# CycloneBoy/pdf_table

Measured on AMD Instinct MI355X. Metric: pages/s, higher is better.
Workload: dtype bf16

## Files before the change

### include/pdftable_hip.h

```cpp
#ifndef PDFTABLE_HIP_H
#define PDFTABLE_HIP_H

#include <stddef.h>
#include <stdint.h>

#ifdef __cplusplus
extern "C" {
#endif

#define PT_OK 0
#define PT_ERR_INVALID 1
#define PT_ERR_HIP 2
#define PT_ERR_STATE 3
#define PT_ERR_FORMAT 4

typedef struct pt_engine pt_engine;
typedef void* pt_stream;

int pt_engine_create(int device_id, pt_engine** out);
void pt_engine_destroy(pt_engine* e);
const char* pt_last_error(void);
int pt_abi_version(void);
int pt_engine_check(pt_engine* e);
int pt_engine_set_lstm_cluster(pt_engine* e, int on);
// ... 170 lines not shown
                 pt_stream stream);
int pt_op_conv1x1_ex(pt_engine* e, const uint16_t* d_in, int B, int H, int W, int Cin, const uint16_t* d_w_tiled, const float* d_bias,
                     int N, uint16_t* d_out, float* d_out_f32, int out_cstride, int n_valid, const float* d_res_f32, int relu,
                     const int32_t* d_ylimit, pt_stream stream);

int pt_op_dcn(pt_engine* e, const uint16_t* d_in, const float* d_om, int B, int H, int W, int C, const uint16_t* d_w_tiled,
              const float* d_bias, int N, uint16_t* d_out, int relu, int split, pt_stream stream);

int pt_op_stem7x7(pt_engine* e, const uint16_t* d_in, int B, int H, int W, const uint16_t* d_w, const float* d_bias,
                  uint16_t* d_out, int split, pt_stream stream);
int pt_op_maxpool3x3s2(pt_engine* e, const uint16_t* d_in, int B, int H, int W, int C, uint16_t* d_out, int split,
                       pt_stream stream);
int pt_op_db_head_final(pt_engine* e, const uint16_t* d_in, int B, int H, int W, const void* d_w, const float* d_bias,
                        float* d_prob, float* d_logits, int split, pt_stream stream);

int pt_op_dwconv(pt_engine* e, const uint16_t* d_in, int B, int H, int W, int C, const float* d_w_taps, const float* d_bias, int k,
                 int stride, int act, uint16_t* d_out, int split, pt_stream stream);
int pt_op_add(pt_engine* e, const uint16_t* d_a, const uint16_t* d_b, uint16_t* d_out, long long npix, int C, int split, pt_stream stream);
int pt_op_maxpool(pt_engine* e, const uint16_t* d_in, int B, int H, int W, int C, int k, int stride, int pad, uint16_t* d_out,
                  int split, pt_stream stream);
int pt_op_avgpool(pt_engine* e, const uint16_t* d_in, int B, int H, int W, int C, int k, uint16_t* d_out, int split, pt_stream stream);
int pt_op_chan_mean(pt_engine* e, const uint16_t* d_in, int B, int HW, int C, float* d_scratch, uint16_t* d_mean, int split, pt_stream stream);
int pt_op_chan_mean_scratch_floats(int B, int C);
int pt_op_scale_channels(pt_engine* e, const uint16_t* d_in, const uint16_t* d_gate, int B, int HW, int C, uint16_t* d_out,
                         int split, pt_stream stream);
int pt_op_act(pt_engine* e, const uint16_t* d_in, long long n_elems, int kind, float alpha, float beta, uint16_t* d_out, int C, int split,
              pt_stream stream);
int pt_op_copy_channels(pt_engine* e, const uint16_t* d_src, long long npix, int src_cstride, int src_coff, uint16_t* d_dst, int dst_cstride, int dst_coff,
                        int n, pt_stream stream);
int pt_op_upsample_nearest(pt_engine* e, const uint16_t* d_in, int B, int H, int W, int C, int factor, uint16_t* d_out, pt_stream stream);
int pt_op_mul(pt_engine* e, const uint16_t* d_a, const uint16_t* d_b, uint16_t* d_out, long long n_elems, int C, int split, pt_stream stream);
int pt_copy_bytes(pt_engine* e, const void* src, void* dst, long long nbytes, pt_stream stream);
int pt_op_layernorm(pt_engine* e, const uint16_t* d_in, long long rows, int c_pad, int c, const float* d_gamma, const float* d_beta, float eps,
                    uint16_t* d_out, int split, pt_stream stream);
int pt_op_softmax(pt_engine* e, const uint16_t* d_in, long long rows, int c_pad, int c, float* d_out_f32, uint16_t* d_out_bf16, int split, pt_stream stream);
int pt_op_attention(pt_engine* e, const uint16_t* d_qkv, int B, int T, int heads, int d, int qkv_cstride, float scale, uint16_t* d_out, int out_cstride,
                    int split, pt_stream stream);

#define PT_CLS_SLOTS 4
#define PT_CLS_MAX_CLASSES 16
typedef struct pt_cls_image {
  int64_t offset;
  int32_t h, w;
} pt_cls_image;

int pt_cls_preprocess(pt_engine* e, const uint8_t* d_base, const pt_cls_image* d_images, int n, int max_h, int max_w,
// ... 50 lines not shown
```

### pdf_table_amd/csrc/api_common.cpp

```cpp
#include <stdarg.h>
#include <stdio.h>

#include "../../include/pdftable_hip.h"

static thread_local char g_err[1024] = "";

void pt_set_error(const char* fmt, ...) {
  va_list ap;
  va_start(ap, fmt);
  vsnprintf(g_err, sizeof(g_err), fmt, ap);
  va_end(ap);
}

extern "C" {

const char* pt_last_error(void) { return g_err; }

int pt_abi_version(void) { return 16; }

}
```

### pdf_table_amd/csrc/c_api.hip

```cpp
#include <stdarg.h>
#include <stdio.h>
#include <stdlib.h>

#include <cmath>

#include "common.h"

namespace PT_FMT_NS {
namespace api {

static int ensure(void** buf, size_t* cap, size_t need);

int pt_engine_check(pt_engine* e) {
  PT_REQUIRE(e, "pt_engine_check: null engine");
  if (e->lstm_err && *e->lstm_err) {
    *e->lstm_err = 0;
    e->lstm_cluster = 0;
    pt_set_error("lstm_cluster_kernel: a workgroup waited > 2^22 polls for its peers -- the launch was not co-resident "
                 "(GPU shared with another process or stream?).  The recognition results since the last check are invalid; "
                 "this engine now uses the streaming LSTM kernel (pt_engine_set_lstm_cluster(e, 0)): run the batch again");
    return PT_ERR_HIP;
  }
  return PT_OK;
}
// ... 910 lines not shown
                 const float* d_bias, int N, int ks, int stride, uint16_t* d_out, int out_cstride, int out_coff,
                 int rep, int shuffle_cout, const uint16_t* d_res, int res_mode, int relu, int split, int out_lo_off,
                 pt_stream stream) {
  PT_REQUIRE(e != nullptr, "pt_op_conv2d: null engine");
  ConvDesc d;
  d.in = d_in; d.B = B; d.H = H; d.W = W; d.Cin = Cin; d.w = d_w_tiled; d.bias = d_bias; d.N = N; d.ks = ks;
  d.stride = stride; d.out = d_out; d.out_cstride = out_cstride; d.out_coff = out_coff; d.rep = rep;
  d.shuffle_cout = shuffle_cout; d.res = d_res; d.res_mode = res_mode; d.relu = relu;
  d.split = split; d.out_lo_off = out_lo_off;
  return pt_launch_conv(e, d, reinterpret_cast<hipStream_t>(stream));
}

int pt_op_conv1x1_ex(pt_engine* e, const uint16_t* d_in, int B, int H, int W, int Cin, const uint16_t* d_w_tiled, const float* d_bias,
                     int N, uint16_t* d_out, float* d_out_f32, int out_cstride, int n_valid, const float* d_res_f32, int relu,
                     const int32_t* d_ylimit, pt_stream stream) {
  PT_REQUIRE(e != nullptr, "pt_op_conv1x1_ex: null engine");
  ConvDesc d;
  d.in = d_in; d.B = B; d.H = H; d.W = W; d.Cin = Cin; d.w = d_w_tiled; d.bias = d_bias; d.N = N; d.ks = 1; d.stride = 1;
  d.out = d_out_f32 ? nullptr : d_out; d.out_f32 = d_out_f32; d.out_cstride = out_cstride; d.n_valid = n_valid; d.res_f32 = d_res_f32;
  d.relu = relu; d.ylimit = d_ylimit;
  return pt_launch_conv(e, d, reinterpret_cast<hipStream_t>(stream));
}

int pt_op_stem7x7(pt_engine* e, const uint16_t* d_in, int B, int H, int W, const uint16_t* d_w, const float* d_bias,
                  uint16_t* d_out, int split, pt_stream stream) {
  PT_REQUIRE(e != nullptr, "pt_op_stem7x7: null engine");
  return pt_launch_stem7x7(e, d_in, B, H, W, d_w, d_bias, d_out, split, reinterpret_cast<hipStream_t>(stream));
}

int pt_op_maxpool3x3s2(pt_engine* e, const uint16_t* d_in, int B, int H, int W, int C, uint16_t* d_out, int split,
                       pt_stream stream) {
  PT_REQUIRE(e && d_in && d_out, "pt_op_maxpool3x3s2: bad arguments");
  return pt_launch_maxpool3x3s2(d_in, B, H, W, C, d_out, split, reinterpret_cast<hipStream_t>(stream));
}

int pt_op_db_head_final(pt_engine* e, const uint16_t* d_in, int B, int H, int W, const void* d_w, const float* d_bias,
                        float* d_prob, float* d_logits, int split, pt_stream stream) {
  PT_REQUIRE(e && d_in && d_w && d_bias && (d_prob || d_logits), "pt_op_db_head_final: bad arguments");
  return pt_launch_db_head_final(d_in, B, H, W, d_w, d_bias, d_prob, d_logits, split, reinterpret_cast<hipStream_t>(stream));
}

int pt_op_dcn(pt_engine* e, const uint16_t* d_in, const float* d_om, int B, int H, int W, int C, const uint16_t* d_w_tiled,
              const float* d_bias, int N, uint16_t* d_out, int relu, int split, pt_stream stream) {
  PT_REQUIRE(e && d_in && d_om && d_w_tiled && d_bias && d_out, "pt_op_dcn: null argument");
  PT_REQUIRE(B > 0 && H > 0 && W > 0, "pt_op_dcn: empty map (B=%d H=%d W=%d)", B, H, W);
  return pt_launch_dcn_fused(e, d_in, d_om, d_w_tiled, d_bias, d_out, B, H, W, C, N, split, relu, reinterpret_cast<hipStream_t>(stream));
// ... 86 lines not shown
```

### pdf_table_amd/csrc/common.h

```cpp
#pragma once
#include <hip/hip_runtime.h>
#include <stdint.h>
#include <string.h>

#include <map>
#include <string>
#include <vector>

#include "../../include/pdftable_hip.h"
#include "act16.h"

typedef uint16_t bf16_t;

void pt_set_error(const char* fmt, ...);

#define PT_HIP_CHECK(expr)                                                                  \
  do {                                                                                      \
    hipError_t _e = (expr);                                                                 \
    if (_e != hipSuccess) {                                                                 \
      pt_set_error("%s failed: %s (%s:%d)", #expr, hipGetErrorString(_e), __FILE__, __LINE__); \
      return PT_ERR_HIP;                                                                    \
    }                                                                                       \
  } while (0)

// ... 278 lines not shown
  int* cols;
  int* glist;
  int* blist3a;
  int* blist2a;
  int* blist2b;
};
int pt_launch_rows_live_list(const int* lim, int n, int* glist, hipStream_t s);
int pt_launch_crnn_limits(const pt_rec_line* lines, int n, const PtCrnnLimits& L, hipStream_t s);
int pt_launch_crnn_fill(bf16_t* out, const bf16_t* ref, const int* lim, int tile_w, int div, int n, int rows, int W, int cs,
                        hipStream_t s, const int* end_lim = nullptr, int end_tile = 1);
int pt_launch_crnn_conv0_pool(const bf16_t* in, int n, int H, int W, const float* w64x9, const float* bias, int split,
                              bf16_t* out, hipStream_t s, const int* xlim = nullptr);
int pt_launch_maxpool_kxk(const bf16_t* in, int n, int H, int W, int C, int kh, int kw, int h2c, int split, bf16_t* out,
                          hipStream_t s);
int pt_launch_lstm(pt_engine* e, const bf16_t* gx, const bf16_t* whh, bf16_t* hout, int B, int T, int split, hipStream_t s);
int pt_launch_gemm_argmax(const bf16_t* A, long long M, int K, const bf16_t* W, const float* bias, int N, int* ids, float* maxv,
                          hipStream_t s);
int pt_launch_gemm_argmax_x3(const bf16_t* A, long long M, int K, const bf16_t* W3, const float* bias, int N, int n_real, int* ids, float* maxv,
                             void* scratch, hipStream_t s);
int pt_launch_gemm_rows_x3(const bf16_t* A, long long M, int K, const bf16_t* W3, const float* bias, int N, bf16_t* out, int relu, hipStream_t s,
                           const int* tlim = nullptr);
int pt_launch_gemm_rows(const bf16_t* A, long long M, int K, const bf16_t* W, const float* bias, int N, bf16_t* out, int relu,
                        hipStream_t s, const int* tlim = nullptr);
int pt_launch_argmax_reduce(const float* part, long long rows, int ntiles, int* ids, float* maxv, hipStream_t s);
int pt_crnn_forward_net(pt_engine* e, const bf16_t* gray, int n, int32_t* ids, float* maxlogit, hipStream_t s,
                        const pt_rec_line* d_lines = nullptr);

int pt_cvit_forward_net(pt_engine* e, const float* gray, int layout, int n, int32_t* ids, float* maxlogit, hipStream_t s,
                        const int* h_text_w = nullptr);
int pt_launch_rec_resize_gray_f32(const uint8_t* crops, const pt_rec_line* lines, const long long* pix_off, int n_lines, int tw,
                                  float* out, hipStream_t s);

int pt_mtl_backbone_forward_net(pt_engine* e, const bf16_t* x, int n, int H, int W, float* f3, hipStream_t s);
void pt_mtl_release(pt_engine* e);
int pt_mtl_preprocess(pt_engine* e, const uint8_t* pages, int ph, int pw, const pt_tsr_table* tabs, int n, int size, bf16_t* out, hipStream_t s);
int pt_mtl_decoder_config(pt_engine* e, int32_t* out13);
int pt_mtl_structure(pt_engine* e, const float* f3, int n, int hw, float* d_tag_logits, float* d_boxes, int32_t* h_lens, int32_t* h_cell_counts,
                     int force_redecode, hipStream_t s);
int pt_mtl_cells(pt_engine* e, int total, int32_t* d_cell_ids, float* d_cell_prob, float* d_cell_logits, int32_t* h_steps, int force_redecode,
                 hipStream_t s);

int pt_db_forward_net(pt_engine* e, const bf16_t* x, int n, int H, int W, float* prob, float* logits, hipStream_t s, uint32_t* bitmap = nullptr,
                      float thresh = 0.f, int* bitmap_done = nullptr);
int pt_launch_tsr_preprocess(const uint8_t* pages, int ph, int pw, const pt_tsr_table* tabs, int n, int H, int W, int bgr,
                             const float* lut, bf16_t* out, int split, hipStream_t s);
int pt_picodet_forward_net(pt_engine* e, const bf16_t* x, int n, int H, int W, float* h0, float* h1, float* h2, float* h3,
// ... 71 lines not shown
```

### pdf_table_amd/csrc/crnn_model.hip

```cpp
#include <stdlib.h>

#include "common.h"

namespace PT_FMT_NS {

namespace {

struct ConvW {
  const PtTensor *w = nullptr, *b = nullptr;
};

int getw(const PtModel& m, const std::string& base, bool x3, ConvW& out) {
  out.w = m.find(base + (x3 ? ".w3" : ".w"));
  out.b = m.find(base + ".b");
  if (!out.w || !out.b) {
    pt_set_error("CRNN weight blob lacks '%s'", base.c_str());
    return PT_ERR_FORMAT;
  }
  return PT_OK;
}

inline const bf16_t* W(const PtTensor* t) { return reinterpret_cast<const bf16_t*>(t->d_ptr); }
inline const float* Bv(const PtTensor* t) { return reinterpret_cast<const float*>(t->d_ptr); }

// ... 81 lines not shown
#define RUN(call) do { if ((rc = (call)) != PT_OK) return rc; } while (0)
  auto conv = [&](const bf16_t* in, int B, int hh, int ww, int cin, const ConvW& cw, int N, int ks, bf16_t* out, int relu) {
    ConvDesc c;
    c.in = in; c.B = B; c.H = hh; c.W = ww; c.Cin = cin; c.w = W(cw.w); c.bias = Bv(cw.b); c.N = N; c.ks = ks;
    c.stride = 1; c.out = out; c.out_cstride = N * m; c.relu = relu; c.split = x3; c.out_lo_off = N;
    return c;
  };
  static int fused = -1;
  if (fused < 0) {
    const char* ev = getenv("PT_CLS_FUSED");
    fused = ev ? atoi(ev) : 1;
  }
  auto rows_x3 = [&]() {
    const char* ev = getenv("PT_ROWS_X3");
    return x3 && fused && !pt_f16x2(e) && !(ev && ev[0] == '0');
  };
  auto gemm_pipe = [&]() {
    const char* ev = getenv("PT_GEMM_PIPE");
    return !x3 && !(ev && ev[0] == '0');
  };
  auto rows_gemm = [&](const bf16_t* in, int cin, const ConvW& cw, int N, bf16_t* out, int relu, const char* label) -> int {
    if (!x3 && fused && (cin == 256 || (cin == 512 && !gemm_pipe()))) {
      PtProfScope ps(e, s, PT_PROF_CONV1X1, 2.0 * n * T * (double)cin * N, label);
      return pt_launch_gemm_rows(in, (long long)n * T, cin, W(cw.w), Bv(cw.b), N, out, relu, s);
    }
    if (rows_x3() && (cin == 512 || cin == 256)) {
      char lb[48];
      snprintf(lb, sizeof(lb), "%s x3", label);
      PtProfScope ps(e, s, PT_PROF_CONV1X1, 2.0 * n * T * (double)cin * N, lb);
      return pt_launch_gemm_rows_x3(in, (long long)n * T, cin, W(cw.w), Bv(cw.b), N, out, relu, s);
    }
    return pt_launch_conv(e, conv(in, 1, n, T, cin, cw, N, 1, out, relu), s);
  };
  int pool_fused = 1;
  {
    const char* ev = getenv("PT_POOL_FUSED");
    if (ev) pool_fused = atoi(ev);
  }
  auto conv_stack = [&](const bf16_t* g, int nn, bf16_t* a0, bf16_t* a1, bf16_t* p1, bf16_t* c2a_o, bf16_t* c2b_o, bf16_t* p2,
                        bf16_t* c3a_o, bf16_t* c3b_o, bf16_t* p3, bf16_t* f_o, bf16_t* gx_o, const PtCrnnLimits* lim,
                        const bf16_t* zl) -> int {
    auto limited = [&](ConvDesc c, int k) {
      if (lim) {
        c.xlimit = lim->lim[k]; c.xlimit_cols = lim->cols + k;
        if (k == 3) c.block_list = lim->blist3a;
        if (k == 4) c.block_list = lim->glist;
// ... 32 lines not shown
      ConvDesc c2d = limited(conv(c2a_o, nn, 8, 160, 256, c2b, 256, 3, p2, 1), 2);
      c2d.pool = 2;
      RUN(pt_launch_conv(e, c2d, s));
      RUN(fill(p2, ZeroLine::P2, 2, 32, 1, 4, 160, 256, 3, 64));
    } else {
      RUN(pt_launch_conv(e, conv(c2a_o, nn, 8, 160, 256, c2b, 256, 3, c2b_o, 1), s));
      RUN(pt_launch_maxpool_kxk(c2b_o, nn, 8, 160, 256, 2, 1, 0, x3, p2, s));
    }
    RUN(pt_launch_conv(e, limited(conv(p2, nn, 4, 160, 256, c3a, 512, 3, c3a_o, 1), 3), s));
    RUN(fill(c3a_o, ZeroLine::C3A, 3, 32, 1, 4, 160, 512, 4, 64));
    if (pool_fused) {
      ConvDesc c3d = limited(conv(c3a_o, nn, 4, 160, 512, c3b, 512, 3, p3, 1), 4);
      c3d.pool = 3;
      RUN(pt_launch_conv(e, c3d, s));
    } else {
      RUN(pt_launch_conv(e, conv(c3a_o, nn, 4, 160, 512, c3b, 512, 3, c3b_o, 1), s));
      RUN(pt_launch_maxpool_kxk(c3b_o, nn, 4, 160, 512, 2, 1, 1, x3, p3, s));
    }
    {
      ConvDesc c4d = conv(p3, 1, nn, T, 1024, c4, 512, 1, f_o, 1);
      if (lim) { c4d.xlimit_rows = lim->lim[4]; c4d.xlimit_cols = lim->cols + 5; c4d.block_list = lim->glist; }
      RUN(pt_launch_conv(e, c4d, s));
    }
    if ((!x3 && fused && !gemm_pipe()) || rows_x3()) {
      int lim_slot = -1;
      {
        PtProfScope ps(e, s, PT_PROF_CONV1X1, 2.0 * nn * T * 512.0 * 2048, x3 ? "rows gemm 512->2048 x3" : "rows gemm 512->2048");
        if (x3) RUN(pt_launch_gemm_rows_x3(f_o, (long long)nn * T, 512, W(xp1.w), Bv(xp1.b), 2048, gx_o, 0, s, lim ? lim->glist : nullptr));
        else RUN(pt_launch_gemm_rows(f_o, (long long)nn * T, 512, W(xp1.w), Bv(xp1.b), 2048, gx_o, 0, s, lim ? lim->glist : nullptr));
        if (lim && ps.idx >= 0 && e->prof.h_lims && e->prof.n_lims < PtProfile::MAX_LIMS) {
          auto& pd = e->prof.pending[ps.idx];
          pd.lim_slot = lim_slot = e->prof.n_lims++;
          pd.rows = nn * T;
        }
      }
      if (lim_slot >= 0) (void)hipMemcpyAsync(e->prof.h_lims + lim_slot, lim->cols + 5, sizeof(int), hipMemcpyDeviceToHost, s);
    } else {
      ConvDesc xd = conv(f_o, 1, nn, T, 512, xp1, 2048, 1, gx_o, 0);
      if (lim) { xd.xlimit_rows = lim->lim[4]; xd.xlimit_cols = lim->cols + 5; xd.block_list = lim->glist; }
      RUN(pt_launch_conv(e, xd, s));
    }
    RUN(fill(gx_o, ZeroLine::GX, 4, 32, 1, 1, 160, 2048, -1, 1));
    return PT_OK;
  };
  const bool ragged = d_lines != nullptr && pool_fused && e->rec_ragged;
  PtCrnnLimits lim;
  const bf16_t* zl = nullptr;
  if (ragged) {
    if (!e->rec_zero_valid[x3]) {
      const size_t bytes = ZeroLine::END * m * sizeof(bf16_t);
      if (!e->rec_zero[x3]) PT_HIP_CHECK(hipMalloc(&e->rec_zero[x3], bytes));
      PT_HIP_CHECK(hipMemsetAsync(e->rec_zero[x3], 0, bytes, s));
      bf16_t* z = reinterpret_cast<bf16_t*>(e->rec_zero[x3]);
      RUN(conv_stack(z + ZeroLine::GRAY * m, 1, z + ZeroLine::A0 * m, nullptr, z + ZeroLine::P1 * m, z + ZeroLine::C2A * m, nullptr,
                     z + ZeroLine::P2 * m, z + ZeroLine::C3A * m, nullptr, z + ZeroLine::P3 * m, z + ZeroLine::F * m,
                     z + ZeroLine::GX * m, nullptr, nullptr));
      e->rec_zero_valid[x3] = true;
      if (!e->rec_zero_ready[x3]) PT_HIP_CHECK(hipEventCreateWithFlags(&e->rec_zero_ready[x3], hipEventDisableTiming));
      PT_HIP_CHECK(hipEventRecord(e->rec_zero_ready[x3], s));
    } else if (e->rec_zero_ready[x3]) {
      PT_HIP_CHECK(hipStreamWaitEvent(s, e->rec_zero_ready[x3], 0));
    }
    zl = reinterpret_cast<const bf16_t*>(e->rec_zero[x3]);
    const size_t need = ((size_t)26 * n + 40) * sizeof(int);
    if (need > e->rec_limits_cap) {
// ... 57 lines not shown
```

### pdf_table_amd/csrc/rec_kernels.hip

```cpp
#include <math.h>

#include "common.h"

namespace PT_FMT_NS {

typedef __attribute__((ext_vector_type(8))) __bf16 bf16x8;
typedef __attribute__((ext_vector_type(16))) float f32x16;
typedef __attribute__((ext_vector_type(4))) uint32_t u32x4;
typedef __attribute__((ext_vector_type(2))) uint32_t u32x2;

__device__ __forceinline__ float rbf2f(uint32_t bits16) { return a16_to_f32(bits16); }
__device__ __forceinline__ uint32_t rf2bf(float f) { return f32_to_a16(f); }

__global__ __launch_bounds__(256) void rec_warp_kernel(const uint8_t* __restrict__ pages, int ph, int pw,
                                                        const pt_rec_line* __restrict__ lines, int n_lines,
                                                        const long long* __restrict__ pix_off, uint8_t* __restrict__ crops) {
  a16_kernel_enter();
  const int li = blockIdx.y;
  if (li >= n_lines) return;
  const pt_rec_line L = lines[li];
  const int cw = L.crop_w, chh = L.crop_h;
  const long long npx = (long long)cw * chh;
  uint8_t* dst = crops + pix_off[li] * 3;
  const uint8_t* src = pages + (size_t)L.page * ph * pw * 3;
// ... 1900 lines not shown
int pt_launch_gemm_rows(const bf16_t* A, long long M, int K, const bf16_t* W, const float* bias, int N, bf16_t* out, int relu,
                        hipStream_t s, const int* tlim) {
  if ((K != 512 && K != 256) || N % 64 != 0 || M <= 0) return PT_ERR_INVALID;
  const int nw = gemm_nw(4);
  const int smem = 64 * (K * 2 + 16) + 64 * 4 + nw * 32 * 80;
  static bool attr_done = false;
  if (!attr_done) {
    PT_HIP_CHECK(hipFuncSetAttribute(reinterpret_cast<const void*>(&gemm_argmax_kernel<32, 1>), hipFuncAttributeMaxDynamicSharedMemorySize, 64 * (512 * 2 + 16) + 256 + 4 * 32 * 80));
    PT_HIP_CHECK(hipFuncSetAttribute(reinterpret_cast<const void*>(&gemm_argmax_kernel<32, 1, 8>), hipFuncAttributeMaxDynamicSharedMemorySize, 64 * (512 * 2 + 16) + 256 + 8 * 32 * 80));
    attr_done = true;
  }
  const dim3 grid((unsigned)((M + nw * 32 - 1) / (nw * 32))), blk(nw * 64);
  if (K == 512) {
    if (nw == 8) hipLaunchKernelGGL((gemm_argmax_kernel<32, 1, 8>), grid, blk, smem, s, A, M, W, bias, N, nullptr, nullptr, out, relu, tlim, 512, 16ll * 2048);
    else hipLaunchKernelGGL((gemm_argmax_kernel<32, 1>), grid, blk, smem, s, A, M, W, bias, N, nullptr, nullptr, out, relu, tlim, 512, 16ll * 2048);
  } else {
    if (nw == 8) hipLaunchKernelGGL((gemm_argmax_kernel<16, 1, 8>), grid, blk, smem, s, A, M, W, bias, N, nullptr, nullptr, out, relu, tlim, 256, 8ll * 2048);
    else hipLaunchKernelGGL((gemm_argmax_kernel<16, 1>), grid, blk, smem, s, A, M, W, bias, N, nullptr, nullptr, out, relu, tlim, 256, 8ll * 2048);
  }
  PT_HIP_CHECK(hipGetLastError());
  return PT_OK;
}

template <int KSTEPS>
__global__ __launch_bounds__(256, KSTEPS == 32 ? 1 : 2) void gemm_rows_x3_kernel(const bf16_t* __restrict__ A, long long M, const bf16_t* __restrict__ W3,
                                                                                 const float* __restrict__ bias, int N, bf16_t* __restrict__ out, int relu,
                                                                                 const int* __restrict__ tlim) {
  a16_kernel_enter();
  constexpr int K = KSTEPS * 16, NCH = K / 32, P = K * 2 + 16;
  constexpr int NPF = NCH;
  extern __shared__ __attribute__((aligned(16))) char smem[];
  char* sw = smem;
  float* sb = reinterpret_cast<float*>(smem + 64 * P);
  const int tid = threadIdx.x, lane = tid & 63, wave = tid >> 6;
  const int lx = lane & 31, q = lane >> 5;
  long long row0 = ((long long)blockIdx.x * 4 + wave) * 32;
  bool live = row0 < M;
  if (tlim) {
    const int total = tlim[0], g = blockIdx.x * 4 + wave;
    if ((int)blockIdx.x * 4 >= total) return;
    live = g < total;
    row0 = live ? (long long)tlim[1 + g] * 32 : 0;
  }
  const long long row = row0 + lx;
  const long long rc = row < M ? row : M - 1;
  bf16x8 ahi[KSTEPS], alo[KSTEPS];
// ... 112 lines not shown
```

### pdf_table_amd/engine.py

```python
from __future__ import annotations

import contextlib
import ctypes as C
import functools
import threading
from typing import Optional, Sequence, Tuple

import numpy as np
import torch

from . import lib as L

__all__ = ["HipEngine", "REC_LINE_DTYPE", "CLS_IMAGE_DTYPE", "REC_PP_ITEM_DTYPE"]

TSR_TABLE_DTYPE = np.dtype([("minv", "<f8", (6,)), ("page", "<i4"), ("x0", "<i4"), ("y0", "<i4"),
                            ("crop_w", "<i4"), ("crop_h", "<i4"), ("reserved", "<i4")])
CLS_IMAGE_DTYPE = np.dtype([("offset", "<i8"), ("h", "<i4"), ("w", "<i4")])
REC_LINE_DTYPE = np.dtype([("minv", np.float64, (9,)), ("page", np.int32), ("crop_w", np.int32), ("crop_h", np.int32),
                           ("reserved", np.int32)])


REC_PP_ITEM_DTYPE = np.dtype([("line", "<i4"), ("resized_w", "<i4"), ("img_w", "<i4"), ("reserved", "<i4"),
                              ("out_off", "<i8")])

# ... 606 lines not shown
        if out is None:
            if shuffle_cout:
                out = torch.empty((B, 2 * Ho, 2 * Wo, shuffle_cout * m), dtype=self.act_dtype, device=self._tdev)
            else:
                out = torch.empty((B, Ho * rep, Wo * rep, N * m), dtype=self.act_dtype, device=self._tdev)
        L.check(self.lib.pt_op_conv2d(self._h, _ptr(x), B, H, W, Cin, _ptr(w_tiled), _ptr(bias), N, ks, stride,
                                      _ptr(out), out.shape[-1], out_coff, rep, shuffle_cout, _ptr(res), res_mode,
                                      int(relu), int(split), out.shape[-1] // 2, self._stream()), "pt_op_conv2d")
        return out

    def op_conv1x1_ex(self, x: torch.Tensor, w_tiled: torch.Tensor, bias: torch.Tensor, relu: int = 0, out_f32: bool = False,
                      n_valid: int = 0, res_f32: Optional[torch.Tensor] = None, ylimit: Optional[torch.Tensor] = None) -> torch.Tensor:
        self._chk(x, self.act_dtype, "x")
        self._chk(bias, torch.float32, "bias")
        B, H, W, Cin = x.shape
        N = bias.numel()
        cs = n_valid or N
        out = torch.zeros((B, H, W, cs), dtype=torch.float32 if out_f32 else self.act_dtype, device=self._tdev)
        L.check(self.lib.pt_op_conv1x1_ex(self._h, _ptr(x), B, H, W, Cin, _ptr(w_tiled), _ptr(bias), N, None if out_f32 else _ptr(out),
                                          _ptr(out) if out_f32 else None, cs, n_valid, _ptr(res_f32), int(relu), _ptr(ylimit),
                                          self._stream()), "pt_op_conv1x1_ex")
        return out

    def op_dcn(self, x: torch.Tensor, om: torch.Tensor, w_tiled: torch.Tensor, bias: torch.Tensor, relu: bool = True, split: int = 0) -> torch.Tensor:
        self._chk(x, self.act_dtype, "x")
        self._chk(om, torch.float32, "om")
        self._chk(bias, torch.float32, "bias")
        B, H, W, Cc = x.shape
        m = 2 if split else 1
        Cc //= m
        if tuple(om.shape) != (B, H, W, 32):
            raise ValueError(f"op_dcn: om must be [B,H,W,32], got {tuple(om.shape)}")
        N = bias.numel()
        out = torch.empty((B, H, W, N * m), dtype=self.act_dtype, device=self._tdev)
        L.check(self.lib.pt_op_dcn(self._h, _ptr(x), _ptr(om), B, H, W, Cc, _ptr(w_tiled), _ptr(bias), N, _ptr(out), int(relu), int(split),
                                   self._stream()), "pt_op_dcn")
        return out

    def op_dwconv(self, x: torch.Tensor, w_taps: torch.Tensor, bias: torch.Tensor, k: int, stride: int = 1, act: int = 0, split: bool = False) -> torch.Tensor:
        self._chk(x, self.act_dtype, "x")
        self._chk(w_taps, torch.float32, "w_taps")
        self._chk(bias, torch.float32, "bias")
        B, H, W, Cc = x.shape
        pad = k // 2
        out = torch.empty((B, (H + 2 * pad - k) // stride + 1, (W + 2 * pad - k) // stride + 1, Cc), dtype=self.act_dtype, device=self._tdev)
        L.check(self.lib.pt_op_dwconv(self._h, _ptr(x), B, H, W, Cc // 2 if split else Cc, _ptr(w_taps), _ptr(bias), k, stride, act, _ptr(out), int(split),
# ... 258 lines not shown
```

### pdf_table_amd/lib.py

```python
from __future__ import annotations

import ctypes as C
import os

_HERE = os.path.dirname(os.path.abspath(__file__))
LIB_PATH = os.environ.get("PT_LIB_PATH") or os.path.join(_HERE, "libpdftable_hip.so")

PT_MODEL_DB_RESNET18 = 1
PT_MODEL_CRNN = 2
PT_MODEL_LORE_DLA34 = 3
PT_MODEL_LORE_PROCESSOR = 4
PT_MODEL_PICODET = 5
PT_MODEL_LORE_RESNET18 = 6
PT_MODEL_DB_NAS = 7
PT_MODEL_PPLCNET = 8
PT_MODEL_CONVNEXT_VIT = 16
PT_MODEL_MTL_BACKBONE = 17
PT_MODEL_MTL_DECODER = 18
PT_MODEL_CENTERNET_DLA34 = 19
PT_CVIT_W, PT_CVIT_CHUNK_W, PT_CVIT_CHUNK_STEP, PT_CVIT_T, PT_CVIT_NCLS = 804, 300, 252, 201, 7644
PT_CLS_SLOTS = 4
PT_CLS_MAX_CLASSES = 16
PT_LAYOUT_HEAD_CS, PT_LAYOUT_CAND_FLOATS = 40, 48
PT_DET_PRE_DB_PP = 0
PT_DET_PRE_DB_TORCH = 1
PT_DET_PRE_NONE = 2
PT_PRECISION_BF16 = 0
PT_PRECISION_BF16X3 = 1
PT_PRECISION_F16X2 = 2
PT_PRECISION_F16 = 3
PT_DET_POST_DB_PP = 0
PT_DET_POST_DB_TORCH = 1
PT_TSR_MAX_CELLS = 3000
PT_CENTERNET_MAX_CELLS = 1000
PT_ROTATE_90_CLOCKWISE, PT_ROTATE_180, PT_ROTATE_90_COUNTERCLOCKWISE = 0, 1, 2
PT_REC_H, PT_REC_W, PT_REC_T, PT_REC_NCLS = 32, 640, 160, 7644
PT_PROF_CLASSES = ("conv3x3", "conv1x1", "stem", "other")
EXPECTED_ABI = 16

_lib = None


class PtError(RuntimeError):
    pass


def _proto(lib):
    vp, i, f, sz = C.c_void_p, C.c_int, C.c_float, C.c_size_t
    ip = C.POINTER(C.c_int)
    P = {
        "pt_engine_create": (i, [i, C.POINTER(vp)]),
        "pt_engine_destroy": (None, [vp]),
        "pt_last_error": (C.c_char_p, []),
        "pt_abi_version": (i, []),
        "pt_engine_check": (i, [vp]),
        "pt_engine_set_precision": (i, [vp, i]),
        "pt_engine_set_lstm_cluster": (i, [vp, i]),
        "pt_engine_set_mtl_kv_fp8": (i, [vp, i]),
        "pt_engine_set_dcn_mfma": (i, [vp, i]),
        "pt_weights_load": (i, [vp, i, vp, sz]),
        "pt_weights_load_device": (i, [vp, i, vp, sz, vp]),
# ... 30 lines not shown
        "pt_layout_forward": (i, [vp, vp, i, i, i, i, i, i, f, i, vp, vp, vp]),
        "pt_tsr_preprocess": (i, [vp, vp, i, i, i, vp, i, i, i, i, vp, vp]),
        "pt_tsr_forward_net": (i, [vp, vp, i, i, i, vp, vp, vp, vp, vp, vp, vp]),
        "pt_tsr_forward_net_wireless": (i, [vp, vp, i, i, i, vp, vp, vp, vp, vp, vp, vp]),
        "pt_tsr_decode": (i, [vp, vp, vp, vp, vp, vp, vp, i, i, i, i, f, vp, vp, vp, vp]),
        "pt_tsr_forward_decode": (i, [vp, vp, i, i, i, i, f, vp, vp, vp, vp]),
        "pt_tsr_process": (i, [vp, vp, vp, vp, i, i, vp, vp, vp]),
        "pt_centernet_forward_net": (i, [vp, vp, i, i, i, vp, vp, vp, vp, vp]),
        "pt_centernet_decode": (i, [vp, vp, vp, vp, vp, i, i, i, vp, vp, vp, vp]),
        "pt_hard_nms": (i, [vp, vp, vp, i, C.c_double, i, vp, vp]),
        "pt_page_line_mask": (i, [vp, i, i, i, vp, vp]),
        "pt_page_line_angles": (i, [vp, i, i, i, i, i, vp, i, vp]),
        "pt_page_warp_cubic": (i, [vp, i, i, i, vp, vp, i, vp, vp]),
        "pt_page_quarter_turn": (i, [vp, i, i, i, i, vp, vp]),
        "pt_page_pre_tables": (i, [vp, vp]),
        "pt_cls_preprocess": (i, [vp, vp, vp, i, i, i, i, i, vp, vp]),
        "pt_cls_forward_net": (i, [vp, i, vp, i, i, i, i, vp, ip, vp]),
        "pt_cls_forward": (i, [vp, i, vp, vp, i, i, i, i, i, i, vp, ip, vp]),
        "pt_cls_forward_lines": (i, [vp, i, vp, i, i, i, vp, vp, i, i, i, i, i, i, vp, ip, vp]),
        "pt_cls_forward_lines_direct": (i, [vp, i, vp, i, i, i, vp, i, i, i, i, i, i, vp, ip, vp]),
        "pt_op_conv2d": (i, [vp, vp, i, i, i, i, vp, vp, i, i, i, vp, i, i, i, i, vp, i, i, i, i, vp]),
        "pt_op_conv1x1_ex": (i, [vp, vp, i, i, i, i, vp, vp, i, vp, vp, i, i, vp, i, vp, vp]),
        "pt_op_dcn": (i, [vp, vp, vp, i, i, i, i, vp, vp, i, vp, i, i, vp]),
        "pt_op_stem7x7": (i, [vp, vp, i, i, i, vp, vp, vp, i, vp]),
        "pt_op_maxpool3x3s2": (i, [vp, vp, i, i, i, i, vp, i, vp]),
        "pt_op_db_head_final": (i, [vp, vp, i, i, i, vp, vp, vp, vp, i, vp]),
        "pt_op_dwconv": (i, [vp, vp, i, i, i, i, vp, vp, i, i, i, vp, i, vp]),
        "pt_op_add": (i, [vp, vp, vp, vp, C.c_longlong, i, i, vp]),
        "pt_op_maxpool": (i, [vp, vp, i, i, i, i, i, i, i, vp, i, vp]),
        "pt_op_avgpool": (i, [vp, vp, i, i, i, i, i, vp, i, vp]),
        "pt_op_chan_mean": (i, [vp, vp, i, i, i, vp, vp, i, vp]),
        "pt_op_chan_mean_scratch_floats": (i, [i, i]),
        "pt_op_scale_channels": (i, [vp, vp, vp, i, i, i, vp, i, vp]),
        "pt_op_act": (i, [vp, vp, C.c_longlong, i, C.c_float, C.c_float, vp, i, i, vp]),
        "pt_op_copy_channels": (i, [vp, vp, C.c_longlong, i, i, vp, i, i, i, vp]),
        "pt_op_upsample_nearest": (i, [vp, vp, i, i, i, i, i, vp, vp]),
        "pt_op_mul": (i, [vp, vp, vp, vp, C.c_longlong, i, i, vp]),
        "pt_copy_bytes": (i, [vp, vp, vp, C.c_longlong, vp]),
        "pt_op_layernorm": (i, [vp, vp, C.c_longlong, i, i, vp, vp, C.c_float, vp, i, vp]),
        "pt_op_softmax": (i, [vp, vp, C.c_longlong, i, i, vp, vp, i, vp]),
        "pt_op_attention": (i, [vp, vp, i, i, i, i, i, C.c_float, vp, i, i, vp]),
        "pt_profile_enable": (i, [vp, i]),
        "pt_profile_read": (i, [vp, vp, vp, vp]),
        "pt_profile_read_labels": (i, [vp, C.c_char_p, i]),
    }
    for name, (res, args) in P.items():
# ... 31 lines not shown
```

Before: 804.5.

## Add wide rows GEMM kernel with fused GX zero-line fill for CRNN

Adds a new rows GEMM kernel for the CRNN 512->2048 input projection. It streams weight tiles into LDS through buffer-load-to-LDS double buffering, keeps A in registers, and stages output through a per-wave LDS transpose so global stores are coalesced. Extra workgroups launched alongside the GEMM perform the per-line GX zero-fill, replacing the separate fill kernel launch. The path is on by default through PT_ROWS_WIDE and is also taken when gemm_pipe is active, which may displace a tuned pipelined path.

```diff
diff --git a/include/pdftable_hip.h b/include/pdftable_hip.h
--- a/include/pdftable_hip.h
+++ b/include/pdftable_hip.h
@@ -216,6 +216,9 @@
 int pt_op_avgpool(pt_engine* e, const uint16_t* d_in, int B, int H, int W, int C, int k, uint16_t* d_out, int split, pt_stream stream);
 int pt_op_chan_mean(pt_engine* e, const uint16_t* d_in, int B, int HW, int C, float* d_scratch, uint16_t* d_mean, int split, pt_stream stream);
 int pt_op_chan_mean_scratch_floats(int B, int C);
+int pt_op_rows_gemm(pt_engine* e, const uint16_t* d_a, long long M, int K, const uint16_t* d_w_tiled, const float* d_bias, int N, uint16_t* d_out,
+                    int kernel, const int32_t* d_lim, int n_lines, int32_t* d_list, const uint16_t* d_fill_ref, pt_stream stream);
+int pt_rows_fill_first_step(int lim, int T);
 int pt_op_scale_channels(pt_engine* e, const uint16_t* d_in, const uint16_t* d_gate, int B, int HW, int C, uint16_t* d_out,
                          int split, pt_stream stream);
 int pt_op_act(pt_engine* e, const uint16_t* d_in, long long n_elems, int kind, float alpha, float beta, uint16_t* d_out, int C, int split,
diff --git a/pdf_table_amd/csrc/api_common.cpp b/pdf_table_amd/csrc/api_common.cpp
--- a/pdf_table_amd/csrc/api_common.cpp
+++ b/pdf_table_amd/csrc/api_common.cpp
@@ -16,6 +16,6 @@
 
 const char* pt_last_error(void) { return g_err; }
 
-int pt_abi_version(void) { return 16; }
+int pt_abi_version(void) { return 17; }
 
 }
diff --git a/pdf_table_amd/csrc/c_api.hip b/pdf_table_amd/csrc/c_api.hip
--- a/pdf_table_amd/csrc/c_api.hip
+++ b/pdf_table_amd/csrc/c_api.hip
@@ -956,6 +956,22 @@
   return pt_launch_conv(e, d, reinterpret_cast<hipStream_t>(stream));
 }
 
+int pt_op_rows_gemm(pt_engine* e, const uint16_t* d_a, long long M, int K, const uint16_t* d_w_tiled, const float* d_bias, int N, uint16_t* d_out,
+                    int kernel, const int32_t* d_lim, int n_lines, int32_t* d_list, const uint16_t* d_fill_ref, pt_stream stream) {
+  PT_REQUIRE(e && d_a && d_w_tiled && d_bias && d_out && (kernel == 0 || kernel == 1), "pt_op_rows_gemm: bad arguments");
+  PT_REQUIRE(!d_lim || (d_list && n_lines > 0 && M == (long long)n_lines * PT_REC_T), "pt_op_rows_gemm: limits need the list buffer and M = n_lines * 160");
+  PT_REQUIRE(!d_fill_ref || d_lim, "pt_op_rows_gemm: a fill needs limits");
+  hipStream_t s = reinterpret_cast<hipStream_t>(stream);
+  int rc;
+  if (d_lim && (rc = pt_launch_rows_live_list(d_lim, n_lines, d_list, s)) != PT_OK) return rc;
+  if (kernel == 1) return pt_launch_gemm_rows_wide(d_a, M, K, d_w_tiled, d_bias, N, d_out, 0, s, d_lim ? d_list : nullptr, d_fill_ref ? d_lim : nullptr, d_fill_ref, n_lines, PT_REC_T);
+  if ((rc = pt_launch_gemm_rows(d_a, M, K, d_w_tiled, d_bias, N, d_out, 0, s, d_lim ? d_list : nullptr)) != PT_OK) return rc;
+  if (d_fill_ref) return pt_launch_crnn_fill(d_out, d_fill_ref, d_lim, 32, 1, n_lines, 1, PT_REC_T, N, s);
+  return PT_OK;
+}
+
+int pt_rows_fill_first_step(int lim, int T) { return pt_rows_fill_first(lim, T); }
+
 int pt_op_stem7x7(pt_engine* e, const uint16_t* d_in, int B, int H, int W, const uint16_t* d_w, const float* d_bias,
                   uint16_t* d_out, int split, pt_stream stream) {
   PT_REQUIRE(e != nullptr, "pt_op_stem7x7: null engine");
diff --git a/pdf_table_amd/csrc/common.h b/pdf_table_amd/csrc/common.h
--- a/pdf_table_amd/csrc/common.h
+++ b/pdf_table_amd/csrc/common.h
@@ -324,6 +324,14 @@
                            const int* tlim = nullptr);
 int pt_launch_gemm_rows(const bf16_t* A, long long M, int K, const bf16_t* W, const float* bias, int N, bf16_t* out, int relu,
                         hipStream_t s, const int* tlim = nullptr);
+int pt_launch_gemm_rows_wide(const bf16_t* A, long long M, int K, const bf16_t* W, const float* bias, int N, bf16_t* out, int relu, hipStream_t s,
+                             const int* tlim = nullptr, const int* fill_lim = nullptr, const bf16_t* fill_ref = nullptr, int n_lines = 0, int T = 0);
+int pt_rows_wide();
+__host__ __device__ inline int pt_rows_fill_first(int lim, int T) {
+  const int x = (lim + 31) / 32 * 32;
+  return x < T ? x : T;
+}
+inline int pt_rows_fill_wgs(int n_lines) { return n_lines < 1 ? 1 : (n_lines < 256 ? n_lines : 256); }
 int pt_launch_argmax_reduce(const float* part, long long rows, int ntiles, int* ids, float* maxv, hipStream_t s);
 int pt_crnn_forward_net(pt_engine* e, const bf16_t* gray, int n, int32_t* ids, float* maxlogit, hipStream_t s,
                         const pt_rec_line* d_lines = nullptr);
diff --git a/pdf_table_amd/csrc/crnn_model.hip b/pdf_table_amd/csrc/crnn_model.hip
--- a/pdf_table_amd/csrc/crnn_model.hip
+++ b/pdf_table_amd/csrc/crnn_model.hip
@@ -127,6 +127,7 @@
   auto rows_gemm = [&](const bf16_t* in, int cin, const ConvW& cw, int N, bf16_t* out, int relu, const char* label) -> int {
     if (!x3 && fused && (cin == 256 || (cin == 512 && !gemm_pipe()))) {
       PtProfScope ps(e, s, PT_PROF_CONV1X1, 2.0 * n * T * (double)cin * N, label);
+      if (N == 2048 && pt_rows_wide() == 2) return pt_launch_gemm_rows_wide(in, (long long)n * T, cin, W(cw.w), Bv(cw.b), N, out, relu, s);
       return pt_launch_gemm_rows(in, (long long)n * T, cin, W(cw.w), Bv(cw.b), N, out, relu, s);
     }
     if (rows_x3() && (cin == 512 || cin == 256)) {
@@ -205,11 +206,16 @@
       if (lim) { c4d.xlimit_rows = lim->lim[4]; c4d.xlimit_cols = lim->cols + 5; c4d.block_list = lim->glist; }
       RUN(pt_launch_conv(e, c4d, s));
     }
-    if ((!x3 && fused && !gemm_pipe()) || rows_x3()) {
+    const bool wide = !x3 && fused && pt_rows_wide() != 0;
+    const char* evf = getenv("PT_GX_FILL_FUSED");
+    const bool gx_fill_fused = wide && lim && !(evf && evf[0] == '0');
+    if ((!x3 && fused && (!gemm_pipe() || wide)) || rows_x3()) {
       int lim_slot = -1;
       {
         PtProfScope ps(e, s, PT_PROF_CONV1X1, 2.0 * nn * T * 512.0 * 2048, x3 ? "rows gemm 512->2048 x3" : "rows gemm 512->2048");
         if (x3) RUN(pt_launch_gemm_rows_x3(f_o, (long long)nn * T, 512, W(xp1.w), Bv(xp1.b), 2048, gx_o, 0, s, lim ? lim->glist : nullptr));
+        else if (wide) RUN(pt_launch_gemm_rows_wide(f_o, (long long)nn * T, 512, W(xp1.w), Bv(xp1.b), 2048, gx_o, 0, s, lim ? lim->glist : nullptr,
+                                                    gx_fill_fused ? lim->lim[4] : nullptr, gx_fill_fused ? zl + ZeroLine::GX * m : nullptr, nn, T));
         else RUN(pt_launch_gemm_rows(f_o, (long long)nn * T, 512, W(xp1.w), Bv(xp1.b), 2048, gx_o, 0, s, lim ? lim->glist : nullptr));
         if (lim && ps.idx >= 0 && e->prof.h_lims && e->prof.n_lims < PtProfile::MAX_LIMS) {
           auto& pd = e->prof.pending[ps.idx];
@@ -223,7 +229,7 @@
       if (lim) { xd.xlimit_rows = lim->lim[4]; xd.xlimit_cols = lim->cols + 5; xd.block_list = lim->glist; }
       RUN(pt_launch_conv(e, xd, s));
     }
-    RUN(fill(gx_o, ZeroLine::GX, 4, 32, 1, 1, 160, 2048, -1, 1));
+    if (!gx_fill_fused) RUN(fill(gx_o, ZeroLine::GX, 4, 32, 1, 1, 160, 2048, -1, 1));
     return PT_OK;
   };
   const bool ragged = d_lines != nullptr && pool_fused && e->rec_ragged;
diff --git a/pdf_table_amd/csrc/rec_kernels.hip b/pdf_table_amd/csrc/rec_kernels.hip
--- a/pdf_table_amd/csrc/rec_kernels.hip
+++ b/pdf_table_amd/csrc/rec_kernels.hip
@@ -1946,6 +1946,188 @@
   return PT_OK;
 }
 
+template <int KSTEPS, int MT, int NW>
+__global__ __launch_bounds__(NW * 64, MT == 2 ? 2 : 1) void gemm_rows_wide_kernel(const bf16_t* __restrict__ A, long long M, const bf16_t* __restrict__ W,
+                                                                                 const float* __restrict__ bias, int N, bf16_t* __restrict__ out, int relu,
+                                                                                 const int* __restrict__ tlim, const int* __restrict__ fill_lim,
+                                                                                 const bf16_t* __restrict__ fill_ref, int n_lines, int T) {
+#if defined(__HIP_DEVICE_COMPILE__)
+  a16_kernel_enter();
+  constexpr int K = KSTEPS * 16, NCH = K / 32, P = 1040, LROWS = 64 * K * 2 / 1024, TILE = LROWS * P, D = 2, NTHR = NW * 64;
+  constexpr int HALF1 = K == 512 ? 32 * P : 512;
+  constexpr int XP = 144, XT = 16 * XP;
+  constexpr int NST = MT * 4;
+  static_assert(LROWS % NW == 0 && LROWS / NW == 8, "eight DMA requests per wave and tile");
+  extern __shared__ __attribute__((aligned(16))) char smem[];
+  float* sb = reinterpret_cast<float*>(smem + 2 * TILE);
+  const int tid = threadIdx.x, lane = tid & 63;
+  const int wave = __builtin_amdgcn_readfirstlane(tid >> 6);
+  const int lx = lane & 31, q = lane >> 5;
+  int nwg = gridDim.x;
+  int total = 0;
+  if (tlim) {
+    total = tlim[0];
+    nwg = (total + NW * MT - 1) / (NW * MT);
+  }
+  if ((int)blockIdx.x >= nwg) {
+    if (!fill_lim) return;
+    const int d = blockIdx.x - nwg, nd = gridDim.x - nwg, pc = N >> 3;
+    const u32x4* r = reinterpret_cast<const u32x4*>(fill_ref);
+    for (int b = d; b < n_lines; b += nd) {
+      const int xf = pt_rows_fill_first(fill_lim[b], T);
+      u32x4* o = reinterpret_cast<u32x4*>(out + (size_t)b * T * N);
+      for (int i = xf * pc + tid; i < T * pc; i += NTHR) o[i] = r[i];
+    }
+    return;
+  }
+  long long row0[MT];
+  bool live[MT];
+  bool full = true;
+#pragma unroll
+  for (int m = 0; m < MT; ++m) {
+    const int g = ((int)blockIdx.x * NW + wave) * MT + m;
+    live[m] = true;
+    row0[m] = (long long)g * 32;
+    if (tlim) {
+      live[m] = g < total;
+      row0[m] = live[m] ? (long long)tlim[1 + g] * 32 : 0;
+    } else if (row0[m] >= M) {
+      live[m] = false;
+      row0[m] = 0;
+    }
+    full = full && live[m] && row0[m] + 32 <= M;
+  }
+  bf16x8 areg[MT][KSTEPS];
+#pragma unroll
+  for (int m = 0; m < MT; ++m) {
+    const long long row = row0[m] + lx, rc = row < M ? row : M - 1;
+#pragma unroll
+    for (int ks = 0; ks < KSTEPS; ++ks) areg[m][ks] = *reinterpret_cast<const bf16x8*>(A + rc * K + ks * 16 + q * 8);
+  }
+  constexpr int OOB = 0x7FFFF000;
+  const __amdgpu_buffer_rsrc_t r_w = __builtin_amdgcn_make_buffer_rsrc(const_cast<bf16_t*>(W), 0, OOB, 0x00020000);
+  int voff[8];
+#pragma unroll
+  for (int j = 0; j < 8; ++j) {
+    const int r = wave + NW * j;
+    if (K == 512) voff[j] = ((((lane >> 2) * 64 + r) * 32) + (lane & 3) * 8) * 2;
+    else voff[j] = ((((lane & 31) >> 2) * 64 + r + 32 * (lane >> 5)) * 32 + (lane & 3) * 8) * 2;
+  }
+  const int NT = N / 64;
+  constexpr int WTS = NCH * 2048 * 2;
+  if (tid < 64) sb[tid] = bias[tid];
+#pragma unroll
+  for (int j = 0; j < 8; ++j)
+    __builtin_amdgcn_raw_ptr_buffer_load_lds(r_w, (__attribute__((address_space(3))) void*)(smem + (wave + NW * j) * P), 16, voff[j], 0, 0, 0);
+  asm volatile("s_waitcnt vmcnt(0)\n\ts_waitcnt lgkmcnt(0)" ::: "memory");
+  __builtin_amdgcn_s_barrier();
+  char* xt = smem + 2 * TILE + 512 + wave * XT;
+  for (int t = 0; t < NT; ++t) {
+    const int b = t & 1;
+    const bool more = t + 1 < NT;
+    const int soff = more ? (t + 1) * WTS : 0;
+    float pb = 0.f;
+    if (tid < 64) pb = bias[(more ? t + 1 : t) * 64 + tid];
+#pragma unroll
+    for (int j = 0; j < 8; ++j)
+      __builtin_amdgcn_raw_ptr_buffer_load_lds(r_w, (__attribute__((address_space(3))) void*)(smem + (b ^ 1) * TILE + (wave + NW * j) * P), 16,
+                                               more ? voff[j] : OOB, soff, 0, 0);
+    const char* wr = smem + b * TILE + lx * P + q * 16;
+    if (live[0]) {
+      f32x16 acc[MT][2];
+#pragma unroll
+      for (int m = 0; m < MT; ++m)
+#pragma unroll
+        for (int r = 0; r < 16; ++r) { acc[m][0][r] = 0.f; acc[m][1][r] = 0.f; }
+      bf16x8 f0[D + 1], f1[D + 1];
+#pragma unroll
+      for (int d = 0; d < D; ++d) {
+        f0[d] = *reinterpret_cast<const bf16x8*>(wr + d * 32);
+        f1[d] = *reinterpret_cast<const bf16x8*>(wr + HALF1 + d * 32);
+      }
+#pragma unroll
+      for (int ks = 0; ks < KSTEPS; ++ks) {
+        if (ks + D < KSTEPS) {
+          f0[(ks + D) % (D + 1)] = *reinterpret_cast<const bf16x8*>(wr + (ks + D) * 32);
+          f1[(ks + D) % (D + 1)] = *reinterpret_cast<const bf16x8*>(wr + HALF1 + (ks + D) * 32);
+        }
+#pragma unroll
+        for (int m = 0; m < MT; ++m) {
+          acc[m][0] = mfma_32x32x16_a16(f0[ks % (D + 1)], areg[m][ks], acc[m][0]);
+          acc[m][1] = mfma_32x32x16_a16(f1[ks % (D + 1)], areg[m][ks], acc[m][1]);
+        }
+      }
+      const float* sbt = sb + b * 64;
+#pragma unroll
+      for (int m = 0; m < MT; ++m) {
+        if (!live[m]) continue;
+        u32x2 pk[2][4];
+#pragma unroll
+        for (int h = 0; h < 2; ++h)
+#pragma unroll
+          for (int rg = 0; rg < 4; ++rg) {
+            const int cl = h * 32 + rg * 8 + 4 * q;
+            float v[4];
+#pragma unroll
+            for (int k = 0; k < 4; ++k) {
+              v[k] = acc[m][h][rg * 4 + k] + sbt[cl + k];
+              if (relu == 1) v[k] = fmaxf(v[k], 0.f);
+              else if (relu == 4) v[k] = gelu_poly(v[k]);
+            }
+            pk[h][rg] = u32x2{pack_a16x2(v[0], v[1]), pack_a16x2(v[2], v[3])};
+          }
+#pragma unroll
+        for (int p = 0; p < 2; ++p) {
+          if ((lx >> 4) == p) {
+#pragma unroll
+            for (int h = 0; h < 2; ++h)
+#pragma unroll
+              for (int rg = 0; rg < 4; ++rg) *reinterpret_cast<u32x2*>(xt + (lx & 15) * XP + (h * 32 + rg * 8 + 4 * q) * 2) = pk[h][rg];
+          }
+          asm volatile("s_waitcnt lgkmcnt(0)" ::: "memory");
+#pragma unroll
+          for (int i = 0; i < 2; ++i) {
+            const int r = (lane >> 3) + 8 * i;
+            const u32x4 v = *reinterpret_cast<const u32x4*>(xt + r * XP + (lane & 7) * 16);
+            const long long row = row0[m] + 16 * p + r;
+            if (full || row < M) *reinterpret_cast<u32x4*>(out + row * N + t * 64 + (lane & 7) * 8) = v;
+          }
+          asm volatile("s_waitcnt lgkmcnt(0)" ::: "memory");
+        }
+      }
+    }
+    if (tid < 64) sb[(b ^ 1) * 64 + tid] = pb;
+    if (full) asm volatile("s_waitcnt vmcnt(%0)\n\ts_waitcnt lgkmcnt(0)" ::"n"(NST) : "memory");
+    else asm volatile("s_waitcnt vmcnt(0)\n\ts_waitcnt lgkmcnt(0)" ::: "memory");
+    __builtin_amdgcn_s_barrier();
+  }
+#endif
+}
+
+int pt_rows_wide() {
+  const char* ev = getenv("PT_ROWS_WIDE");
+  return ev ? (ev[0] == '0' ? 0 : (ev[0] == '2' ? 2 : 1)) : 1;
+}
+
+int pt_launch_gemm_rows_wide(const bf16_t* A, long long M, int K, const bf16_t* W, const float* bias, int N, bf16_t* out, int relu, hipStream_t s,
+                             const int* tlim, const int* fill_lim, const bf16_t* fill_ref, int n_lines, int T) {
+  if ((K != 512 && K != 256) || N % 64 != 0 || M <= 0) return PT_ERR_INVALID;
+  if (fill_lim) PT_REQUIRE(fill_ref && tlim && n_lines > 0 && T % 32 == 0 && (long long)n_lines * T == M, "rows gemm: the fill needs the live list and whole lines");
+  constexpr int SMEM512 = 2 * 64 * 1040 + 512 + 8 * 16 * 144, SMEM256 = 2 * 32 * 1040 + 512 + 4 * 16 * 144;
+  static bool attr_done = false;
+  if (!attr_done) {
+    PT_HIP_CHECK(hipFuncSetAttribute(reinterpret_cast<const void*>(&gemm_rows_wide_kernel<32, 1, 8>), hipFuncAttributeMaxDynamicSharedMemorySize, SMEM512));
+    PT_HIP_CHECK(hipFuncSetAttribute(reinterpret_cast<const void*>(&gemm_rows_wide_kernel<16, 2, 4>), hipFuncAttributeMaxDynamicSharedMemorySize, SMEM256));
+    attr_done = true;
+  }
+  const long long groups = (M + 31) >> 5;
+  const unsigned nwg = (unsigned)((groups + 7) / 8) + (fill_lim ? pt_rows_fill_wgs(n_lines) : 0);
+  if (K == 512) hipLaunchKernelGGL((gemm_rows_wide_kernel<32, 1, 8>), dim3(nwg), dim3(512), SMEM512, s, A, M, W, bias, N, out, relu, tlim, fill_lim, fill_ref, n_lines, T);
+  else hipLaunchKernelGGL((gemm_rows_wide_kernel<16, 2, 4>), dim3(nwg), dim3(256), SMEM256, s, A, M, W, bias, N, out, relu, tlim, fill_lim, fill_ref, n_lines, T);
+  PT_HIP_CHECK(hipGetLastError());
+  return PT_OK;
+}
+
 template <int KSTEPS>
 __global__ __launch_bounds__(256, KSTEPS == 32 ? 1 : 2) void gemm_rows_x3_kernel(const bf16_t* __restrict__ A, long long M, const bf16_t* __restrict__ W3,
                                                                                  const float* __restrict__ bias, int N, bf16_t* __restrict__ out, int relu,
diff --git a/pdf_table_amd/engine.py b/pdf_table_amd/engine.py
--- a/pdf_table_amd/engine.py
+++ b/pdf_table_amd/engine.py
@@ -652,6 +652,21 @@
                                           self._stream()), "pt_op_conv1x1_ex")
         return out
 
+    def op_rows_gemm(self, a: torch.Tensor, w_tiled: torch.Tensor, bias: torch.Tensor, kernel: int = 1, lim: Optional[torch.Tensor] = None,
+                     fill_ref: Optional[torch.Tensor] = None, out: Optional[torch.Tensor] = None) -> torch.Tensor:
+        self._chk(a, self.act_dtype, "a")
+        self._chk(bias, torch.float32, "bias")
+        M, K = a.shape
+        N = bias.numel()
+        if out is None:
+            out = torch.zeros((M, N), dtype=self.act_dtype, device=self._tdev)
+        n_lines = 0 if lim is None else lim.numel()
+        lst = None if lim is None else torch.zeros((1 + 5 * n_lines,), dtype=torch.int32, device=self._tdev)
+        L.check(self.lib.pt_op_rows_gemm(self._h, _ptr(a), M, K, _ptr(w_tiled), _ptr(bias), N, _ptr(out), int(kernel), _ptr(lim), n_lines, _ptr(lst),
+                                         _ptr(fill_ref), self._stream()), "pt_op_rows_gemm")
+        torch.cuda.synchronize()
+        return out
+
     def op_dcn(self, x: torch.Tensor, om: torch.Tensor, w_tiled: torch.Tensor, bias: torch.Tensor, relu: bool = True, split: int = 0) -> torch.Tensor:
         self._chk(x, self.act_dtype, "x")
         self._chk(om, torch.float32, "om")
diff --git a/pdf_table_amd/lib.py b/pdf_table_amd/lib.py
--- a/pdf_table_amd/lib.py
+++ b/pdf_table_amd/lib.py
@@ -36,7 +36,7 @@
 PT_ROTATE_90_CLOCKWISE, PT_ROTATE_180, PT_ROTATE_90_COUNTERCLOCKWISE = 0, 1, 2
 PT_REC_H, PT_REC_W, PT_REC_T, PT_REC_NCLS = 32, 640, 160, 7644
 PT_PROF_CLASSES = ("conv3x3", "conv1x1", "stem", "other")
-EXPECTED_ABI = 16
+EXPECTED_ABI = 17
 
 _lib = None
 
@@ -113,6 +113,8 @@
         "pt_op_conv2d": (i, [vp, vp, i, i, i, i, vp, vp, i, i, i, vp, i, i, i, i, vp, i, i, i, i, vp]),
         "pt_op_conv1x1_ex": (i, [vp, vp, i, i, i, i, vp, vp, i, vp, vp, i, i, vp, i, vp, vp]),
         "pt_op_dcn": (i, [vp, vp, vp, i, i, i, i, vp, vp, i, vp, i, i, vp]),
+        "pt_op_rows_gemm": (i, [vp, vp, C.c_longlong, i, vp, vp, i, vp, i, vp, i, vp, vp, vp]),
+        "pt_rows_fill_first_step": (i, [i, i]),
         "pt_op_stem7x7": (i, [vp, vp, i, i, i, vp, vp, vp, i, vp]),
         "pt_op_maxpool3x3s2": (i, [vp, vp, i, i, i, i, vp, i, vp]),
         "pt_op_db_head_final": (i, [vp, vp, i, i, i, vp, vp, vp, vp, i, vp]),
```

Result: no change. 806.5 (median of 5 runs) (+0.2%).
